# Orange-OpenSource/AIVC

Measured on AMD Instinct MI355X. Metric: encode+decode fps @1080p YUV420 (RA GOP32), higher is better.
Workload: dtype f32; 1 GPU; 1920x1080 8-bit YUV420, coding structure 1_GOP_32: one 128-frame clip = 4 intra-period units of 33 frames (132 coded frames, the last 4 repeat the last frame) encoded + decoded per step; synthetic random-init stand-in for model ms_ssim-4 (widths {'n2': 64, 'n': 128, 'c_y': 64, 'c_short': 64, 'c_z': 32, 'n_h': 128}), last analysis conv calibrated so that 6 (MOFNet) / 12 (CodecNet) of the 64 y featu; parallelism=single GPU

## Files before the change

### aivc_amd/abi.py

```python
import ctypes as C

ABI_VERSION = 23
PREC_FP32, PREC_BF16X3, PREC_FP32_WINO = 0, 1, 2

AIVC_OK = 0
ERR_UNSUPPORTED = -2
ERRORS = {0: 'AIVC_OK', -1: 'AIVC_ERR_ARG', -2: 'AIVC_ERR_UNSUPPORTED', -3: 'AIVC_ERR_LAUNCH',
          -4: 'AIVC_ERR_WORKSPACE'}

MODE_CONV, MODE_TCONV, MODE_GDN, MODE_IGDN = 0, 1, 2, 3
ACT_NONE, ACT_LEAKY, ACT_RELU, ACT_SIGMOID = 0, 1, 2, 3
ALGO_AUTO, ALGO_DIRECT, ALGO_MFMA = 0, 1, 2

AC_MAX_VAL = 256
LP = 514
CDF_ROW = 520
CDF_WIN0, CDF_WIN = 224, 64
BALLE_PARAMS = 43
MAX_MAPS = 256
RC_MAX_STREAMS = 64
RATE_LANES = 16384
SSE_BLOCKS = 64
WINO_MIN_PIXELS = 8000
WINO_MIN_PIXELS_TCONV = 32768
# ... 121 lines not shown
DETMATH_EXPF, DETMATH_EXPM1F, DETMATH_SIGMOIDF, DETMATH_TANHF, DETMATH_SOFTPLUSF = 4, 5, 6, 7, 8
DETMATH_POWF, DETMATH_LAPLACE_CDF = 9, 10
DETMATH_COUNT = 11


def detmath_is_fp64(fn):
    return DETMATH_EXP <= fn <= DETMATH_LOG1P


def detmath_operands(fn):
    return 2 if fn in (DETMATH_POWF, DETMATH_LAPLACE_CDF) else 1

COLOR_PROTOTYPES = {
    'aivc_rgb8_to_yuv420u8': [_f, _i32, _i32, _i32, _f, _f, _f],
    'aivc_yuv8_to_rgb8': [_f, _f, _f, _i32, _i32, _i32, _i32, _i32, _i32, _f],
}

QUALITY_PROTOTYPES = {
    'aivc_frame_sse_u8': [_f, _f, _f, _f, _f, _f, _i32, _i32, _i32, _f, _f],
    'aivc_frame_aux_stats': [_f, _f, _f, _f, _i32, _i32, _i32, _i32, _i32, _i32, _f, _f],
}

RATES_PROTOTYPES = {
    'aivc_channel_gain_rows': [_f, _f, _i32, _sz, _i32, _f],
    'aivc_quantize_center_rows': [_f, _f, _f, _i32, _sz, _i32, _f, _f],
    'aivc_dequantize_rows': [_f, _f, _f, _i32, _sz, _i32, _f],
}

DIGEST_PROTOTYPES = {
    'aivc_md5_batch': [_f, C.c_int64, _i32, _f],
}


def declare(lib, suffix=''):
    fns = {}
    for name, args in PROTOTYPES.items():
        fn = getattr(lib, name + suffix)
        fn.argtypes = list(args) + [C.c_void_p]
        fn.restype = C.c_int
        fns[name] = fn
    if not suffix:
        var = lib.aivc_conv2d_variant
        var.argtypes = [_P(ConvParams)]
        var.restype = C.c_int
        fns['aivc_conv2d_variant'] = var
        chk = lib.aivc_selfcheck_gdn_math
        chk.argtypes = [C.c_uint64, C.c_uint32, _f, C.c_void_p]
        chk.restype = C.c_int
        fns['aivc_selfcheck_gdn_math'] = chk
        ev = lib.aivc_detmath_eval
        ev.argtypes = list(DETMATH_EVAL_ARGS) + [C.c_void_p]
        ev.restype = C.c_int
        fns['aivc_detmath_eval'] = ev
        wm = lib.aivc_warp_modes
        wm.argtypes = [_f, _f, _i32, _i32, _i32, _i32, _i32, _i32, _i32, _f, C.c_void_p]
        wm.restype = C.c_int
        fns['aivc_warp_modes'] = wm
        for name, args in list(COLOR_PROTOTYPES.items()) + list(QUALITY_PROTOTYPES.items()) + list(RATES_PROTOTYPES.items()) \
                + list(DIGEST_PROTOTYPES.items()):
            fn = getattr(lib, name)
            fn.argtypes = list(args) + [C.c_void_p]
            fn.restype = C.c_int
            fns[name] = fn
    mws = getattr(lib, 'aivc_metrics_workspace' + suffix)
    mws.argtypes = [_i32, _i32, _i32]
    mws.restype = C.c_size_t
    fns['aivc_metrics_workspace'] = mws
    ver = getattr(lib, 'aivc_abi_version' + suffix)
    ver.argtypes = []
    ver.restype = C.c_int
    fns['aivc_abi_version'] = ver
    return fns


def conv_out_size(mode, h, w, k, stride, pad):
    if mode == MODE_CONV:
        return (h + 2 * pad - k) // stride + 1, (w + 2 * pad - k) // stride + 1
    if mode == MODE_TCONV:
        return 2 * h, 2 * w
    return h, w
```

### aivc_amd/csrc/conv_wino.hip

```cpp
#include <stdlib.h>

#include "mfma_util.h"
#include "wino_class_walk.h"

namespace aivc {

struct WinoArgs {
  aivc_conv_params p;
  int TH, TW;
  int nby, nbx;
  int gy;
  int total;
  int poly;
  int cpp_shift;
};

constexpr int WINO_RAW_STAGE = 11 * 1024;
constexpr int WINO_U_STAGE = 32 * 1024;
constexpr int WINO_V_QUAD = 1152;
constexpr int WINO_V_POS = 2 * WINO_V_QUAD;
constexpr int WINO_V_STAGE = 16 * WINO_V_POS;
constexpr int WINO_LDS = 2 * (WINO_RAW_STAGE + WINO_U_STAGE + WINO_V_STAGE);

__device__ __attribute__((aligned(4096))) float wino_zeros[1024];

template <int MODE>
__host__ __device__ constexpr bool wino_zero_pos(int pc, int i, int j) {
  if constexpr (MODE == 1) return ((pc >> 1) && i == 3) || ((pc & 1) && j == 3);
  if constexpr (MODE == 2) return ((pc >> 1) && i == 0) || ((pc & 1) && j == 0);
  return false;
}
template <int MODE>
__host__ __device__ constexpr uint32_t wino_pos_mask(int pc, int half) {
  uint32_t m = 0u;
  for (int q = 0; q < 8; ++q) m |= wino_zero_pos<MODE>(pc, 2 * half + (q >> 2), q & 3) ? 0u : 1u << q;
  return m;
}

struct WinoWalk {
  uint32_t x_lo, x_hi, slot, wg_per_xcd;
  __device__ __forceinline__ WinoWalk(uint32_t total, uint32_t nwg, uint32_t wg) {
    const uint32_t xcd = wg & 7u;
    slot = wg >> 3;
    const uint32_t per_xcd = (total + 7u) >> 3;
    wg_per_xcd = (nwg + 7u - xcd) >> 3;
    x_lo = xcd * per_xcd;
    x_hi = min(x_lo + per_xcd, total);
  }
  __device__ __forceinline__ uint32_t block_of(uint32_t k) const { return x_lo + slot + k * wg_per_xcd; }
  __device__ __forceinline__ uint32_t count() const { return x_lo + slot < x_hi ? (x_hi - x_lo - slot + wg_per_xcd - 1u) / wg_per_xcd : 0u; }
};

template <int MODE>
__global__ __launch_bounds__(512) void conv_wino_kernel(WinoArgs a) {
  constexpr bool POLY = MODE == 1, TC = MODE == 2;
  extern __shared__ __attribute__((aligned(16))) char wsmem[];
  char *raw = wsmem, *Us = wsmem + 2 * WINO_RAW_STAGE, *Vs = Us + 2 * WINO_U_STAGE;
  const uint32_t lds0 = (uint32_t)(uintptr_t)(__attribute__((address_space(3))) char *)wsmem;

  const aivc_conv_params &p = a.p;
  const int tid = threadIdx.x, lane = tid & 63;
  const int wave = __builtin_amdgcn_readfirstlane(tid >> 6);
  const int ph = wave >> 2, wm = (wave >> 1) & 1, wn = wave & 1;
  const int H = TC ? p.h_in : p.h_out, W = TC ? p.w_in : p.w_out, Hi = p.h_in, Wi = p.w_in, Cin = p.c_in, Cout = p.c_out;
  const int gyc = TC ? 4 * a.gy : a.gy;
  const int cpp_shift = a.cpp_shift, cpp_mask = (1 << a.cpp_shift) - 1;

  const WinoWalk walk((uint32_t)a.total, gridDim.x, blockIdx.x);
  const uint32_t n_mine = walk.count();
  if (n_mine == 0u) return;
  struct Desc {
    const float *xbase, *ubase;
    uint32_t r_off[2];
    int img, byi, bxi, cb;
  };
  int s_quad[2], s_py[2], s_px[2];
#pragma unroll
  for (int k = 0; k < 2; ++k) {
    int sl = 64 * (wave + 8 * k) + lane;
    sl = sl < 648 ? sl : 647;
    const int q2 = sl >> 1, plane = q2 / 81, rem = q2 - plane * 81, hy = rem / 9, hx = rem - hy * 9;
    s_quad[k] = sl & 1;
    s_py[k] = 2 * hy + (plane >> 1);
    s_px[k] = 2 * hx + (plane & 1);
  }
  const int nch = POLY ? 4 * (Cin >> 3) : (Cin >> 3);
  auto make_desc = [&](uint32_t blk) {
    Desc d;
    uint32_t rest;
    if constexpr (TC) {
      const WinoClassEntry e = wino_class_entry(blk, (uint32_t)gyc, (uint32_t)a.total, gridDim.x);
      d.cb = (int)e.cb;
      rest = e.pb;
    } else {
      d.cb = (int)(blk % (uint32_t)gyc);
      rest = blk / (uint32_t)gyc;
    }
    d.bxi = (int)(rest % (uint32_t)a.nbx);
    rest /= (uint32_t)a.nbx;
    d.byi = (int)(rest % (uint32_t)a.nby);
    d.img = (int)(rest / (uint32_t)a.nby);
    d.xbase = p.x + (size_t)d.img * (size_t)Hi * Wi * Cin;
    d.ubase = p.w_wino + (size_t)d.cb * (size_t)nch * (WINO_U_STAGE / 4);
    if constexpr (MODE == 0) {
#pragma unroll
      for (int k = 0; k < 2; ++k) {
        const int iy = max(min(16 * d.byi - 1 + s_py[k], Hi - 1), 0), ix = max(min(16 * d.bxi - 1 + s_px[k], Wi - 1), 0);
        d.r_off[k] = ((uint32_t)(iy * Wi + ix) * (uint32_t)Cin + (uint32_t)(4 * s_quad[k])) * 4u;
      }
    }
    return d;
  };
  uint32_t iss_off[2];
  auto patch_offsets = [&](const Desc &d_, int ph2) {
    const int st = POLY ? 2 : 1, py = ph2 >> 1, px = ph2 & 1;
#pragma unroll
    for (int k = 0; k < 2; ++k) {
      const int iy = max(min(st * (16 * d_.byi - 1 + s_py[k]) + py, Hi - 1), 0), ix = max(min(st * (16 * d_.bxi - 1 + s_px[k]) + px, Wi - 1), 0);
      iss_off[k] = ((uint32_t)(iy * Wi + ix) * (uint32_t)Cin + (uint32_t)(4 * s_quad[k])) * 4u;
    }
  };
  uint64_t iss_addr[2];
  auto tc_addresses = [&](const Desc &d_) {
#pragma unroll
    for (int k = 0; k < 2; ++k) {
      const int iy = 16 * d_.byi - 1 + s_py[k], ix = 16 * d_.bxi - 1 + s_px[k];
      const bool in = iy >= 0 && iy < Hi && ix >= 0 && ix < Wi;
      const uint64_t a_in = (uint64_t)(uintptr_t)d_.xbase + ((uint64_t)((uint32_t)(iy * Wi + ix)) * (uint32_t)Cin + (uint32_t)(4 * s_quad[k])) * 4u;
      const uint64_t a_z = (uint64_t)(uintptr_t)wino_zeros + (uint32_t)(16 * s_quad[k]);
      iss_addr[k] = in ? a_in : a_z;
    }
  };
  Desc cur = make_desc(walk.block_of(0)), nxt = n_mine > 1u ? make_desc(walk.block_of(1)) : cur;

  const uint32_t r_dst = __builtin_amdgcn_readfirstlane(lds0 + (uint32_t)wave * 1024u);
  const uint32_t u_dst = __builtin_amdgcn_readfirstlane(lds0 + (uint32_t)(2 * WINO_RAW_STAGE) + (uint32_t)wave * 4096u);
  const uint32_t u_off = (uint32_t)(wave * 4096 + lane * 16);
  auto uniform_ptr = [](const float *q) -> const float * {
    const uint64_t v = (uint64_t)(uintptr_t)q;
    const uint32_t lo = __builtin_amdgcn_readfirstlane((uint32_t)v), hi = __builtin_amdgcn_readfirstlane((uint32_t)(v >> 32));
    return reinterpret_cast<const float *>((uintptr_t)(((uint64_t)hi << 32) | lo));
  };
  auto issue_raw = [&](const Desc &d_, int c) {
    const uint32_t d = r_dst + (uint32_t)((c & 1) * WINO_RAW_STAGE);
    if constexpr (TC) {
      if (c == 0) tc_addresses(d_);
      const uint32_t du = __builtin_amdgcn_readfirstlane(d);
      asm volatile("s_mov_b32 m0, %1\n\ts_nop 0\n\tglobal_load_lds_dwordx4 %0, off" : : "v"(iss_addr[0]), "s"(du) : "memory", "m0");
      if (wave < 3) asm volatile("s_mov_b32 m0, %1\n\ts_nop 0\n\tglobal_load_lds_dwordx4 %0, off" : : "v"(iss_addr[1]), "s"(du + 8192u) : "memory", "m0");
      iss_addr[0] += 32u;
      iss_addr[1] += 32u;
    } else {
      const float *src = d_.xbase + 8 * c;
      glds16(src, d_.r_off[0], d);
      if (wave < 3) glds16(src, d_.r_off[1], d + 8192u);
    }
  };
  auto issue_u = [&](const Desc &d_, int c) {
    const float *src = TC ? uniform_ptr(d_.ubase + (size_t)c * (WINO_U_STAGE / 4)) : d_.ubase + (size_t)c * (WINO_U_STAGE / 4);
    const uint32_t d = TC ? __builtin_amdgcn_readfirstlane(u_dst + (uint32_t)((c & 1) * WINO_U_STAGE)) : u_dst + (uint32_t)((c & 1) * WINO_U_STAGE);
    bool lo = true, hi = true;
    if constexpr (TC) {
      const int cls = d_.cb / a.gy, i = wave >> 1, j = 2 * (wave & 1);
      lo = !wino_zero_pos<MODE>(cls, i, j);
      hi = !wino_zero_pos<MODE>(cls, i, j + 1);
    }
    if (lo && hi) glds_piece<GLDS_BOTH>(src, u_off, d);
    else if (lo) glds_piece<GLDS_LO>(src, u_off, d);
    else if (hi) glds_piece<GLDS_HI>(src, u_off, d);
  };

  struct Prep {
    const float *r_src, *u_src;
    uint32_t flags;
  };
  auto prepare = [&](uint32_t kb, int cr, int cu) -> Prep {
    Prep q;
    const bool more = kb + 1u < n_mine;
    uint32_t fl = 0u;
    {
      const bool own = cr < nch;
      const int c = own ? cr : cr - nch;
      const Desc &d_ = own ? cur : nxt;
      if (own || more) {
        fl |= 1u;
        if ((c & cpp_mask) == 0) patch_offsets(d_, c >> cpp_shift);
      }
      q.r_src = uniform_ptr(d_.xbase + 8 * (c & cpp_mask));
    }
    {
      const bool own = cu < nch;
      const int c = own ? cu : cu - nch;
      const Desc &d_ = own ? cur : nxt;
      q.u_src = uniform_ptr(d_.ubase + (size_t)c * (WINO_U_STAGE / 4));
      if (own || more) {
        const int pc = c >> cpp_shift, i = wave >> 1, j = 2 * (wave & 1);
        if (!wino_zero_pos<MODE>(pc, i, j)) fl |= 2u;
        if (!wino_zero_pos<MODE>(pc, i, j + 1)) fl |= 4u;
      }
    }
    q.flags = __builtin_amdgcn_readfirstlane(fl);
    return q;
  };
  auto fire_raw = [&](auto STAGE, const Prep &q) {
    const uint32_t d = r_dst + (uint32_t)(decltype(STAGE)::value * WINO_RAW_STAGE);
    if (q.flags & 1u) {
      glds16(q.r_src, iss_off[0], d);
      if (wave < 3) glds16(q.r_src, iss_off[1], d + 8192u);
    }
  };
  auto fire_u = [&](auto STAGE, const Prep &q) {
    const uint32_t d = u_dst + (uint32_t)(decltype(STAGE)::value * WINO_U_STAGE);
    const uint32_t both = q.flags & 6u;
    if (both == 6u) glds_piece<GLDS_BOTH>(q.u_src, u_off, d);
    else if (both == 2u) glds_piece<GLDS_LO>(q.u_src, u_off, d);
    else if (both == 4u) glds_piece<GLDS_HI>(q.u_src, u_off, d);
  };

  const int l32 = lane & 31;
  const int t_grp = (l32 < 4 || (l32 >= 12 && l32 < 16) || (l32 >= 20 && l32 < 28)) ? 0 : 1;
  const int t_pos = t_grp == 0 ? (l32 < 4 ? l32 : (l32 < 16 ? l32 - 8 : l32 - 12)) : (l32 < 12 ? l32 - 4 : (l32 < 20 ? l32 - 8 : l32 - 16));
  const int t_quad = t_pos >> 3, t_tx = (t_pos & 7) ^ (t_grp << 2), t_ty = ((tid >> 6) & 1) * 4 + (lane >> 5) * 2 + t_grp;
  const int t_i = __builtin_amdgcn_readfirstlane(tid >> 7);
  const int t_ra = t_i == 0 ? 0 : (t_i == 2 ? 2 : 1), t_rb = t_i == 3 ? 3 : (t_i == 2 ? 1 : 2);
  const float t_si = t_i == 1 ? 1.0f : -1.0f;
  const int t_base = ((t_ty * 9 + t_tx) * 2 + t_quad) * 16;
  auto pix_off = [](int r, int c) { return (((r & 1) * 2 + (c & 1)) * 81 + (r >> 1) * 9 + (c >> 1)) * 32; };
  int t_oa[4], t_ob[4];
#pragma unroll
  for (int c = 0; c < 4; ++c) {
    t_oa[c] = t_base + pix_off(t_ra, c);
// ... 75 lines not shown
        const char *rs = raw + (1 - stage) * WINO_RAW_STAGE;
        ta[0] = *reinterpret_cast<const float4 *>(rs + t_oa[st]);
        tb[0] = *reinterpret_cast<const float4 *>(rs + t_ob[st]);
        ta[1] = *reinterpret_cast<const float4 *>(rs + t_oa[st + 1]);
        tb[1] = *reinterpret_cast<const float4 *>(rs + t_ob[st + 1]);
      };
      auto finish = [&](auto S) {
        constexpr int st = decltype(S)::value;
        if constexpr (st < 4) {
          R[st] = comb(ta[0], tb[0], t_si);
          R[st + 1] = comb(ta[1], tb[1], t_si);
        } else {
          transform_step(NEXT{}, integral_constant<int, st>{});
          transform_step(NEXT{}, integral_constant<int, st + 1>{});
        }
      };
      if constexpr (q < 4) reads(Q);
      __builtin_amdgcn_sched_barrier(0);
      const float4 x0 = af[set][0], y0 = bf[set][0], x1 = af[set][1], y1 = bf[set][1];
      if constexpr (first && TC) {
        const floatx16 zero = {0.0f, 0.0f, 0.0f, 0.0f, 0.0f, 0.0f, 0.0f, 0.0f, 0.0f, 0.0f, 0.0f, 0.0f, 0.0f, 0.0f, 0.0f, 0.0f};
        if ((pm >> q) & 1u) acc[q] = mfma_oct1(x0, y0, zero);
        else acc[q] = __builtin_amdgcn_mfma_f32_32x32x2f32(0.0f, 0.0f, zero, 0, 0, 0);
        if ((pm >> (q + 1)) & 1u) acc[q + 1] = mfma_oct1(x1, y1, zero);
        else acc[q + 1] = __builtin_amdgcn_mfma_f32_32x32x2f32(0.0f, 0.0f, zero, 0, 0, 0);
      } else if constexpr (first) {
        const floatx16 zero = {0.0f, 0.0f, 0.0f, 0.0f, 0.0f, 0.0f, 0.0f, 0.0f, 0.0f, 0.0f, 0.0f, 0.0f, 0.0f, 0.0f, 0.0f, 0.0f};
        acc[q] = __builtin_amdgcn_mfma_f32_32x32x2f32(x0.x, y0.x, zero, 0, 0, 0);
        acc[q + 1] = __builtin_amdgcn_mfma_f32_32x32x2f32(x1.x, y1.x, zero, 0, 0, 0);
        acc[q] = __builtin_amdgcn_mfma_f32_32x32x2f32(x0.y, y0.y, acc[q], 0, 0, 0);
        acc[q + 1] = __builtin_amdgcn_mfma_f32_32x32x2f32(x1.y, y1.y, acc[q + 1], 0, 0, 0);
        acc[q] = __builtin_amdgcn_mfma_f32_32x32x2f32(x0.z, y0.z, acc[q], 0, 0, 0);
        acc[q + 1] = __builtin_amdgcn_mfma_f32_32x32x2f32(x1.z, y1.z, acc[q + 1], 0, 0, 0);
        acc[q] = __builtin_amdgcn_mfma_f32_32x32x2f32(x0.w, y0.w, acc[q], 0, 0, 0);
        acc[q + 1] = __builtin_amdgcn_mfma_f32_32x32x2f32(x1.w, y1.w, acc[q + 1], 0, 0, 0);
      } else {
        if (MODE == 0 || ((pm >> q) & 1u)) acc[q] = mfma_oct1(x0, y0, acc[q]);
        if (MODE == 0 || ((pm >> (q + 1)) & 1u)) acc[q + 1] = mfma_oct1(x1, y1, acc[q + 1]);
      }
      __builtin_amdgcn_sched_barrier(0);
      if constexpr (!TC && q == 0) {
        if (!ph) dma();
      }
      finish(Q);
      __builtin_amdgcn_sched_barrier(0);
    };
    using std::integral_constant;
    pair(integral_constant<int, 0>{});
    pair(integral_constant<int, 2>{});
    pair(integral_constant<int, 4>{});
    pair(integral_constant<int, 6>{});
  };

  auto issue_raw_at = [&](uint32_t kb, int c) {
    if (c < nch) issue_raw(cur, c);
    else if (kb + 1u < n_mine) issue_raw(nxt, c - nch);
  };
  auto issue_u_at = [&](uint32_t kb, int c) {
    if (c < nch) issue_u(cur, c);
    else if (kb + 1u < n_mine) issue_u(nxt, c - nch);
  };
  if constexpr (POLY) {
    const Prep q0 = prepare(0u, 0, 0);
    fire_raw(std::integral_constant<int, 0>{}, q0);
    fire_u(std::integral_constant<int, 0>{}, q0);
    fire_raw(std::integral_constant<int, 1>{}, prepare(0u, 1, 0));
  } else {
    issue_raw(cur, 0);
    issue_u(cur, 0);
    issue_raw_at(0u, 1);
  }
  asm volatile("s_waitcnt vmcnt(0)" ::: "memory");
  __builtin_amdgcn_s_barrier();
  transform0();
  asm volatile("s_waitcnt lgkmcnt(0)" ::: "memory");
  __builtin_amdgcn_s_barrier();
  const int act1 = p.act1, act2 = p.act2;
  for (uint32_t kb = 0; kb < n_mine; ++kb) {
    auto chunk = [&](auto STAGE, auto FIRST, int c) {
      Prep q;
      if constexpr (POLY) q = prepare(kb, c + 2, c + 1);
      auto dma = [&]() {
        if constexpr (POLY) {
          fire_raw(STAGE, q);
          fire_u(std::integral_constant<int, 1 - decltype(STAGE)::value>{}, q);
        } else {
          issue_raw_at(kb, c + 2);
          issue_u_at(kb, c + 1);
        }
      };
      uint32_t pm = 0xFFu;
      if constexpr (MODE != 0) {
        constexpr uint32_t ZCOL = 0xFFu ^ wino_pos_mask<MODE>(1, 0), ZROW = 0xFFu ^ wino_pos_mask<MODE>(2, POLY ? 1 : 0);
        static_assert(wino_pos_mask<MODE>(1, 1) == (0xFFu ^ ZCOL) && wino_pos_mask<MODE>(2, POLY ? 0 : 1) == 0xFFu &&
                      wino_pos_mask<MODE>(3, POLY ? 1 : 0) == (0xFFu ^ (ZCOL | ZROW)), "pm's two terms are the whole rule");
        const int pc = POLY ? c >> cpp_shift : cur.cb / a.gy;
        pm = 0xFFu & ~((pc & 1) ? ZCOL : 0u) & ~(((pc >> 1) && (POLY ? ph : !ph)) ? ZROW : 0u);
      }
      if constexpr (TC) dma();
      multiply(STAGE, FIRST, pm, dma);
      asm volatile("s_waitcnt vmcnt(0) lgkmcnt(0)" ::: "memory");
      __builtin_amdgcn_s_barrier();
    };
    {
      using std::integral_constant;
      using S0 = integral_constant<int, 0>;
      using S1 = integral_constant<int, 1>;
      chunk(S0{}, std::true_type{}, 0);
      chunk(S1{}, std::false_type{}, 1);
      for (int c = 2; c < nch; c += 2) {
        chunk(S0{}, std::false_type{}, c);
        chunk(S1{}, std::false_type{}, c + 1);
      }
    }

    floatx16 keep[2], give[2];
    auto fold = [&](auto PH) {
      constexpr int phc = decltype(PH)::value;
#pragma unroll
      for (int bb = 0; bb < 2; ++bb)
#pragma unroll
        for (int r = 0; r < 16; ++r) keep[bb][r] = give[bb][r] = 0.0f;
#pragma unroll
      for (int q = 0; q < 8; ++q) {
        const int i = 2 * phc + (q >> 2), j = q & 3;
        const int t0i = i < 3 ? 1 : 0, t1i = i == 0 ? 0 : (i == 1 ? 1 : -1);
        const int t0j = j < 3 ? 1 : 0, t1j = j == 0 ? 0 : (j == 1 ? 1 : -1);
#pragma unroll
        for (int o = 0; o < 4; ++o) {
          const int cf = ((o >> 1) ? t1i : t0i) * ((o & 1) ? t1j : t0j);
          floatx16 &dst = (o >> 1) == phc ? keep[o & 1] : give[o & 1];
          if (cf > 0) {
#pragma unroll
            for (int r = 0; r < 16; ++r) dst[r] = dst[r] + acc[q][r];
          } else if (cf < 0) {
#pragma unroll
            for (int r = 0; r < 16; ++r) dst[r] = dst[r] - acc[q][r];
          }
        }
      }
    };
    if (ph) fold(std::integral_constant<int, 1>{});
    else fold(std::integral_constant<int, 0>{});
    {
      float *xch = reinterpret_cast<float *>(Vs + WINO_V_STAGE) + wave * 1024;
      const float *theirs = reinterpret_cast<const float *>(Vs + WINO_V_STAGE) + (wave ^ 4) * 1024;
#pragma unroll
      for (int bb = 0; bb < 2; ++bb) {
#pragma unroll
        for (int r = 0; r < 16; ++r) xch[r * 64 + lane] = give[bb][r];
        asm volatile("s_waitcnt lgkmcnt(0)" ::: "memory");
        __builtin_amdgcn_s_barrier();
#pragma unroll
        for (int r = 0; r < 16; ++r) keep[bb][r] = keep[bb][r] + theirs[r * 64 + lane];
        asm volatile("s_waitcnt lgkmcnt(0)" ::: "memory");
        __builtin_amdgcn_s_barrier();
      }
    }

    {
      const float *__restrict__ g_mul = p.mul;
      const float *__restrict__ g_res = p.res;
// ... 54 lines not shown
                if (ok[rr * 2 + b]) *reinterpret_cast<gfloat *>(yb + lane_b + (uint32_t)((2 * rr + b) * 512) * (sx / 512u)) = v;
              }
          }
        };
        using std::integral_constant;
        int kind = -1;
        if (act1 == AIVC_ACT_NONE && act2 == AIVC_ACT_NONE) kind = 0;
        else if (act2 == AIVC_ACT_NONE) kind = act1 == AIVC_ACT_LEAKY ? 1 : 2;
        else if (act1 == AIVC_ACT_NONE) kind = act2 == AIVC_ACT_RELU ? 3 : 4;
        if (kind >= 0 && sx % 512u == 0u) {
          auto go = [&](auto RES, auto INSIDE) {
            switch (kind) {
              case 0: rows(RES, integral_constant<int, 0>{}, INSIDE); break;
              case 1: rows(RES, integral_constant<int, 1>{}, INSIDE); break;
              case 2: rows(RES, integral_constant<int, 2>{}, INSIDE); break;
              case 3: rows(RES, integral_constant<int, 3>{}, INSIDE); break;
              default: rows(RES, integral_constant<int, 4>{}, INSIDE); break;
            }
          };
          if (inside_x) {
            if (g_res) go(integral_constant<bool, true>{}, integral_constant<bool, true>{});
            else go(integral_constant<bool, false>{}, integral_constant<bool, true>{});
          } else {
            if (g_res) go(integral_constant<bool, true>{}, integral_constant<bool, false>{});
            else go(integral_constant<bool, false>{}, integral_constant<bool, false>{});
          }
          goto epilogue_done;
        }
      }
      {
        const size_t ybase = (size_t)cur.img * (size_t)Ho_ * Wo_ * Cout + (size_t)co;
#pragma unroll
        for (int r = 0; r < 16; ++r) {
          const int t = (r & 3) + 8 * (r >> 2) + 4 * hh;
          const int oy = oy_w + 2 * (t >> 3), ox0 = 2 * (8 * cur.bxi + (t & 7));
          if (oy >= H) continue;
#pragma unroll
          for (int b = 0; b < 2; ++b) {
            const int ox = ox0 + b;
            if (ox >= W) continue;
            const size_t o = ybase + ((size_t)(OS * oy + pyc) * Wo_ + (size_t)(OS * ox + pxc)) * (size_t)Cout;
            float v = keep[b][r];
            if (has_bias) v = v + cbias;
            v = act_cheap(act1, v);
            if (g_mul) v = g_mul[o] * v;
            if (g_res) v = v + g_res[o];
            v = act_cheap(act2, v);
            g_y[o] = v;
          }
        }
      }
    epilogue_done:;
    }
    cur = nxt;
    if (kb + 2u < n_mine) nxt = make_desc(walk.block_of(kb + 2u));
  }
}

__device__ __forceinline__ void wino_g(double g0, double g1, double g2, double (&out)[4]) {
  out[0] = g0;
  out[1] = 0.5 * ((g0 + g1) + g2);
  out[2] = 0.5 * ((g0 - g1) + g2);
  out[3] = g2;
}

struct WinoForm3x3 {
  static constexpr int COUNT = 1;
  int co, ci, c_in;
  __device__ WinoForm3x3(size_t idx, int, int c_in_) : co((int)(idx / c_in_)), ci((int)(idx % c_in_)), c_in(c_in_) {}
  __device__ double tap(const float *w, int r, int l) const { return (double)w[(((size_t)co * 3 + r) * 3 + l) * c_in + ci]; }
  __device__ size_t out(int pos) const { return AIVC_WINO_U_INDEX(co, pos, ci, c_in); }
};
__device__ __forceinline__ double wino_tap5(const float *w, int co, int ci, int c_in, int ky, int kx) {
  return ky < 5 && kx < 5 ? (double)w[(((size_t)co * 5 + ky) * 5 + kx) * c_in + ci] : 0.0;
}
struct WinoFormPoly5 {
  static constexpr int COUNT = 4;
  int co, ci, c_in, phase;
  __device__ WinoFormPoly5(size_t idx, int, int c_in_)
      : co((int)(idx / ((size_t)4 * c_in_))), ci((int)((idx / 4) % c_in_)), c_in(c_in_), phase((int)(idx % 4)) {}
  __device__ double tap(const float *w, int r, int l) const { return wino_tap5(w, co, ci, c_in, 2 * r + (phase >> 1), 2 * l + (phase & 1)); }
  __device__ size_t out(int pos) const { return AIVC_WINO_U_INDEX(co, pos, phase * c_in + ci, 4 * c_in); }
};
struct WinoFormTconv5 {
  static constexpr int COUNT = 4;
  int co, ci, c_in, c_out, cls;
  __device__ WinoFormTconv5(size_t idx, int c_out_, int c_in_)
      : co((int)((idx / c_in_) % c_out_)), ci((int)(idx % c_in_)), c_in(c_in_), c_out(c_out_), cls((int)(idx / ((size_t)c_in_ * c_out_))) {}
  __device__ double tap(const float *w, int r, int l) const { return wino_tap5(w, co, ci, c_in, (cls >> 1) + 4 - 2 * r, (cls & 1) + 4 - 2 * l); }
  __device__ size_t out(int pos) const { return AIVC_WINO_U_INDEX(cls * c_out + co, pos, ci, c_in); }
};

template <class FORM>
__global__ void __launch_bounds__(256) winograd_weights_kernel(const float *w, int c_out, int c_in, float *u) {
  const size_t idx = (size_t)blockIdx.x * 256 + threadIdx.x;
  if (idx >= (size_t)c_out * c_in * FORM::COUNT) return;
  const FORM f(idx, c_out, c_in);
  double t[4][3], uu[4][4];
#pragma unroll
  for (int l = 0; l < 3; ++l) {
    double col[4];
    wino_g(f.tap(w, 0, l), f.tap(w, 1, l), f.tap(w, 2, l), col);
#pragma unroll
    for (int i = 0; i < 4; ++i) t[i][l] = col[i];
  }
#pragma unroll
  for (int i = 0; i < 4; ++i) wino_g(t[i][0], t[i][1], t[i][2], uu[i]);
#pragma unroll
  for (int i = 0; i < 4; ++i)
#pragma unroll
    for (int j = 0; j < 4; ++j) u[f.out(4 * i + j)] = (float)uu[i][j];
}

template <class FORM>
static int winograd_weights_launch(const char *what, const float *w, int c_out, int c_in, float *u, hipStream_t s) {
  hipLaunchKernelGGL(winograd_weights_kernel<FORM>, dim3(cdiv((size_t)c_out * c_in * FORM::COUNT, 256)), dim3(256), 0, s, w, c_out, c_in, u);
  return check_launch(what);
}
int winograd_weights(const float *w, int c_out, int c_in, float *u, hipStream_t s) {
  return winograd_weights_launch<WinoForm3x3>("winograd_weights", w, c_out, c_in, u, s);
}
int winograd_weights_poly5(const float *w, int c_out, int c_in, float *u, hipStream_t s) {
  return winograd_weights_launch<WinoFormPoly5>("winograd_weights_poly5", w, c_out, c_in, u, s);
}
int winograd_weights_tconv5(const float *w, int c_out, int c_in, float *u, hipStream_t s) {
  return winograd_weights_launch<WinoFormTconv5>("winograd_weights_tconv5", w, c_out, c_in, u, s);
}

struct WinoGrid {
  int gh, gw, nby, nbx;
  uint64_t blocks;
};
static WinoGrid wino_grid(const aivc_conv_params &p) {
  const bool tc = p.mode == AIVC_MODE_TCONV;
  const int gh = tc ? p.h_in : p.h_out, gw = tc ? p.w_in : p.w_out, nby = (gh + 15) / 16, nbx = (gw + 15) / 16;
  return {gh, gw, nby, nbx, (uint64_t)p.n * nby * nbx * ((uint64_t)p.c_out / 64) * (tc ? 4 : 1)};
}

bool conv2d_wino_supported(const aivc_conv_params &p) {
  if (!aivc_winograd_covers(&p) || p.gdn) return false;
  if ((uint64_t)p.h_in * p.w_in * p.c_in * 4u >= 0xFFFF0000ull) return false;
  if (p.mode == AIVC_MODE_TCONV && p.c_in > 960) return false;
  return wino_grid(p).blocks < 0x7FFFFFFFull;
}

int conv2d_wino_variant(const aivc_conv_params &p) { return p.mode == AIVC_MODE_TCONV ? 303 : (p.ksize == 5 ? 302 : 301); }

template <int MODE>
static int wino_launch(const WinoArgs &a, unsigned grid, hipStream_t s) {
  static LdsOptIn opt_in;
  if (!opt_in.raise(reinterpret_cast<const void *>(conv_wino_kernel<MODE>), WINO_LDS)) return check_launch("conv_wino lds attribute");
  hipLaunchKernelGGL(conv_wino_kernel<MODE>, dim3(grid), dim3(512), WINO_LDS, s, a);
  return check_launch("conv_wino");
}

int conv2d_wino(const aivc_conv_params &p, hipStream_t s) {
  if (!conv2d_wino_supported(p) || !p.w_wino) return AIVC_ERR_UNSUPPORTED;
  const bool tc = p.mode == AIVC_MODE_TCONV;
  WinoArgs a;
  a.p = p;
  a.poly = !tc && p.ksize == 5 ? 1 : 0;
  a.cpp_shift = 0;
  while ((8 << a.cpp_shift) < p.c_in) ++a.cpp_shift;
  const WinoGrid g = wino_grid(p);
  a.TH = (g.gh + 1) / 2;
  a.TW = (g.gw + 1) / 2;
  a.nby = g.nby;
  a.nbx = g.nbx;
  a.gy = p.c_out / 64;
  a.total = (int)g.blocks;
  static std::atomic<int> n_cu{0};
  if (n_cu.load(std::memory_order_relaxed) == 0) {
    int dev = 0, cus = 0;
    n_cu = hipGetDevice(&dev) == hipSuccess && hipDeviceGetAttribute(&cus, hipDeviceAttributeMultiprocessorCount, dev) == hipSuccess && cus > 0 ? cus : 256;
  }
  unsigned grid = (unsigned)n_cu.load(std::memory_order_relaxed);
  if ((unsigned)a.total < grid) grid = (unsigned)a.total;
  if (tc) return wino_launch<2>(a, grid, s);
  return a.poly ? wino_launch<1>(a, grid, s) : wino_launch<0>(a, grid, s);
}

}
```

### aivc_amd/csrc/selfcheck.hip

```cpp
#include "common.h"

namespace aivc {

__global__ __launch_bounds__(256) void selfcheck_sqrt_kernel(uint32_t first, uint32_t last, unsigned long long *bad) {
  unsigned long long n = 0;
  for (uint64_t b = (uint64_t)first + (uint64_t)blockIdx.x * 256 + threadIdx.x; b <= last; b += (uint64_t)gridDim.x * 256) {
    const float s = __uint_as_float((uint32_t)b);
    n += __float_as_uint(sqrt_rn_safe(s)) != __float_as_uint(__builtin_sqrtf(s));
  }
  if (n) atomicAdd(bad, n);
}

__device__ __forceinline__ uint64_t mix64(uint64_t z) {
  z = (z ^ (z >> 30)) * 0xBF58476D1CE4E5B9ull;
  z = (z ^ (z >> 27)) * 0x94D049BB133111EBull;
  return z ^ (z >> 31);
}

__global__ __launch_bounds__(256) void selfcheck_div_kernel(uint64_t n_pairs, uint32_t seed, unsigned long long *bad) {
  unsigned long long n = 0;
  for (uint64_t i = (uint64_t)blockIdx.x * 256 + threadIdx.x; i < n_pairs; i += (uint64_t)gridDim.x * 256) {
    const uint64_t h = mix64(i + ((uint64_t)seed << 32) + 0x9E3779B97F4A7C15ull), h2 = mix64(h);
    const uint32_t ev = 127u - 60u + (uint32_t)((h >> 23) % 120u), ed = 127u - 30u + (uint32_t)((h2 >> 23) % 60u);
    uint32_t mv = (uint32_t)h & 0x7FFFFFu;
    const uint32_t md = (uint32_t)h2 & 0x7FFFFFu;
    if ((i & 3) == 3) mv = (md + (uint32_t)((h >> 50) & 7u) - 3u) & 0x7FFFFFu;
    const float v = __uint_as_float(((uint32_t)(h >> 63) << 31) | (ev << 23) | mv);
    const float d = __uint_as_float((ed << 23) | md);
    n += __float_as_uint(div_rn_safe(v, d)) != __float_as_uint(v / d);
  }
  if (n) atomicAdd(bad, n);
}

}

AIVC_EXPORT int aivc_selfcheck_gdn_math(uint64_t n_div_pairs, uint32_t seed, uint64_t *mismatch, aivc_stream_t stream) {
  if (!mismatch) return AIVC_ERR_ARG;
  hipStream_t s = aivc::to_stream(stream);
  if (hipMemsetAsync(mismatch, 0, 2 * sizeof(uint64_t), s) != hipSuccess) return aivc::check_launch("selfcheck memset");
  const uint32_t first = __builtin_bit_cast(uint32_t, aivc::GDN_SAFE_LO), last = __builtin_bit_cast(uint32_t, aivc::GDN_SAFE_HI);
  hipLaunchKernelGGL(aivc::selfcheck_sqrt_kernel, dim3(4096), dim3(256), 0, s, first, last, reinterpret_cast<unsigned long long *>(mismatch));
  if (n_div_pairs)
    hipLaunchKernelGGL(aivc::selfcheck_div_kernel, dim3(4096), dim3(256), 0, s, n_div_pairs, seed, reinterpret_cast<unsigned long long *>(mismatch) + 1);
  return aivc::check_launch("selfcheck_gdn_math");
}

namespace aivc {

template <typename T>
__global__ __launch_bounds__(256) void detmath_eval_kernel(int fn, const T *__restrict__ a, const T *__restrict__ b, size_t n, T *__restrict__ out) {
  for (size_t i = (size_t)blockIdx.x * 256 + threadIdx.x; i < n; i += (size_t)gridDim.x * 256) {
    if constexpr (sizeof(T) == 8) {
      const double x = a[i];
      double r;
      switch (fn) {
        case AIVC_DETMATH_EXP: r = aivc_det_exp(x); break;
        case AIVC_DETMATH_EXPM1: r = aivc_det_expm1(x); break;
        case AIVC_DETMATH_LOG: r = aivc_det_log(x); break;
        default: r = aivc_det_log1p(x); break;
      }
      out[i] = r;
    } else {
      const float x = a[i];
      float r;
      switch (fn) {
        case AIVC_DETMATH_EXPF: r = aivc_expf_det(x); break;
        case AIVC_DETMATH_EXPM1F: r = aivc_expm1f_det(x); break;
        case AIVC_DETMATH_SIGMOIDF: r = aivc_sigmoidf_det(x); break;
        case AIVC_DETMATH_TANHF: r = aivc_tanhf_det(x); break;
        case AIVC_DETMATH_SOFTPLUSF: r = aivc_softplusf_det(x); break;
        case AIVC_DETMATH_POWF: r = aivc_powf_det(x, b[i]); break;
        default: r = aivc_laplace_cdf(x, b[i]); break;
      }
      out[i] = r;
    }
  }
}

}

AIVC_EXPORT int aivc_detmath_eval(int32_t fn, const void *a, const void *b, size_t n, void *out, aivc_stream_t stream) {
  if (fn < 0 || fn >= AIVC_DETMATH_COUNT) return AIVC_ERR_ARG;
  if (n == 0) return AIVC_OK;
  const bool two = fn == AIVC_DETMATH_POWF || fn == AIVC_DETMATH_LAPLACE_CDF;
  if (!a || !out || (two && !b)) return AIVC_ERR_ARG;
  hipStream_t s = aivc::to_stream(stream);
  const unsigned blocks = aivc::cdiv(n, 256) < 8192u ? aivc::cdiv(n, 256) : 8192u;
  if (fn <= AIVC_DETMATH_LOG1P)
    hipLaunchKernelGGL(aivc::detmath_eval_kernel<double>, dim3(blocks), dim3(256), 0, s, (int)fn, static_cast<const double *>(a),
                       static_cast<const double *>(b), n, static_cast<double *>(out));
  else
    hipLaunchKernelGGL(aivc::detmath_eval_kernel<float>, dim3(blocks), dim3(256), 0, s, (int)fn, static_cast<const float *>(a),
                       static_cast<const float *>(b), n, static_cast<float *>(out));
  return aivc::check_launch("detmath_eval");
}
```

### aivc_amd/ops.py

```python
import ctypes as C
import os

import numpy as np
import torch

from . import abi
from ._lib import AivcNativeError, call, load

FRAME_I, FRAME_P, FRAME_B = abi.FRAME_I, abi.FRAME_P, abi.FRAME_B

PROFILE = None
PROFILE_DIRECT_EQUIVALENT = [0.0, 0.0]
PROFILE_HBM = None


def _hbm_profiled(name, nbytes, launch):
    if PROFILE_HBM is None:
        return launch()
    e0, e1 = torch.cuda.Event(enable_timing=True), torch.cuda.Event(enable_timing=True)
    e0.record()
    launch()
    e1.record()
    PROFILE_HBM.append((name, float(nbytes), e0, e1))

# ... 191 lines not shown
        flags = abi.CONV_SPARSE4 if cmap is not None and all(ci % 4 != 3 for ci in cmap) else 0
        if WINO_ANY_SIZE:
            flags |= abi.CONV_WINO_ANY_SIZE
    ho, wo = abi.conv_out_size(mode, h, w_, k, stride, pad)
    y = torch.empty((n, ho, wo, co2 or co), dtype=torch.float32, device=x.device)
    bias = _dev(bias, torch.float32, 'bias')
    mul = _dev(mul, torch.float32, 'mul')
    res = _dev(res, torch.float32, 'res')
    for t, nm in ((mul, 'mul'), (res, 'res')):
        if t is not None and tuple(t.shape) != tuple(y.shape):
            raise AivcNativeError('conv2d: %s shape %s != output shape %s' % (nm, tuple(t.shape), tuple(y.shape)))
    g_beta, g_gamma, gflag = (None, None, 0) if gdn is None else (gdn[0], gdn[1], 2 if gdn[2] else 1)
    p = abi.ConvParams(mode, k, stride, pad, n, h, w_, c, ho, wo, co, act1, act2, algo, gflag, flags,
                       _p(x), _p(w_ohwi), _p(bias), _p(mul), _p(res), _p(y), _p(g_beta), _p(g_gamma))
    if co2:
        b3 = _dev(tail[1], torch.float32, 'tail bias')
        p.tail_w, p.tail_bias, p.tail_c_out = _p(w3), _p(b3), co2
    p.precision = PRECISION
    if frame_h is not None and PRECISION == abi.PREC_FP32_WINO:
        p.precision, p.flags = slab_contract(p, frame_h)
    variant = load()['aivc_conv2d_variant'](C.byref(p))
    if variant < 0 and (gdn is not None or co2):
        return _two_launches(x, w_ohwi, bias, mode, stride, pad, act1, act2, mul, res, algo, gdn, tail, frame_h)
    w_derived = None
    if variant in _WINO_VARIANTS:
        w_derived = winograd_weights(w_ohwi, transposed=mode == abi.MODE_TCONV)
        p.w_wino = _p(w_derived)
    elif variant >= 1000 and PRESPLIT_WEIGHTS:
        w_derived = split_weights_bf16x3(w_ohwi)
        p.w_bf16x3 = _p(w_derived)
        variant = load()['aivc_conv2d_variant'](C.byref(p))
    _profiled(lambda: call('aivc_conv2d', C.byref(p), _stream()), variant, mode, k, stride, c_real, co, n, h, w_, ho, wo,
              gdn is not None, co2)
    return y


def gdn_reparam(beta, gamma, beta_bound, gamma_bound, pedestal):
    beta = _dev(beta.detach(), torch.float32, 'beta')
    gamma = _dev(gamma.detach(), torch.float32, 'gamma')
    c = beta.shape[0]
    be = torch.empty_like(beta)
    ge = torch.empty_like(gamma)
    call('aivc_gdn_reparam', _p(beta), _p(gamma), c, float(beta_bound), float(gamma_bound),
         float(pedestal), _p(be), _p(ge), _stream())
    return be, ge


def selfcheck_gdn_math(n_div_pairs=1 << 34, seed=1, device=None):
    out = torch.zeros(2, dtype=torch.int64, device=device or torch.device('cuda'))
    call('aivc_selfcheck_gdn_math', int(n_div_pairs), int(seed), _p(out), _stream())
    return tuple(int(v) for v in out.cpu())


def detmath_eval(fn, a, b=None):
    dt = torch.float64 if abi.detmath_is_fp64(fn) else torch.float32
    a, b = _dev(a, dt, 'a'), _dev(b, dt, 'b')
    if abi.detmath_operands(fn) == 2 and (b is None or b.shape != a.shape):
        raise AivcNativeError('aivc_amd.ops.detmath_eval: function %d takes two operands of one shape' % fn)
    out = torch.empty_like(a)
    call('aivc_detmath_eval', int(fn), _p(a), _p(b), a.numel(), _p(out), _stream())
    return out


def gdn(x, beta_eff, gamma_eff, inverse=False, res=None, algo=abi.ALGO_AUTO, frame_h=None):
    c = x.shape[-1]
    mode = abi.MODE_IGDN if inverse else abi.MODE_GDN
    if c % 4 == 0:
        return conv2d(x, gamma_eff.reshape(c, 1, 1, c), beta_eff, mode=mode, res=res, algo=algo, frame_h=frame_h)
    c4 = (c + 3) // 4 * 4
    g = torch.zeros((c4, c4), dtype=torch.float32, device=x.device)
    g[:c, :c] = gamma_eff
    b = torch.ones(c4, dtype=torch.float32, device=x.device)
    b[:c] = beta_eff
    y = conv2d(pad_channels(x, c4), g.reshape(c4, 1, 1, c4), b, mode=mode,
               res=None if res is None else pad_channels(res, c4), algo=algo, frame_h=frame_h)
    return y[..., :c].contiguous()


def yuv420_to_444(y, u, v, c_store=4, c_off=0, out=None):
    u8 = y.dtype == torch.uint8
    dt = torch.uint8 if u8 else torch.float32
    y, u, v = _dev(y, dt, 'y'), _dev(u, dt, 'u'), _dev(v, dt, 'v')
    n, h, w = y.shape
    if out is None:
        full = c_off == 0 and c_store <= 4
        out = (torch.empty if full else torch.zeros)((n, h, w, c_store), dtype=torch.float32, device=y.device)
    zero_pad = 1 if out.shape[-1] >= c_off + 4 else 0
    hc, wc = (h + 1) // 2, (w + 1) // 2
    _hbm_profiled('yuv420_to_444', n * ((h * w + 2 * hc * wc) * (1 if u8 else 4) + h * w * 4 * (3 + zero_pad)),
                  lambda: call('aivc_yuv420u8_to_444' if u8 else 'aivc_yuv420_to_444', _p(y), _p(u), _p(v), n, h, w,
                               _p(out), out.shape[-1], c_off, zero_pad, _stream()))
    return out


_CONV_IMAGES_MAX = 2


def _n_frames(parts):
    return next(p['y'].shape[0] if isinstance(p, dict) else p.shape[0] for p in parts if p is not None)


def _image_sources(parts):
    arr = (abi.ImageSrc * abi.MAX_IMAGES)()
    keep = []
    for i, p in enumerate(parts):
        if isinstance(p, dict):
# ... 664 lines not shown
```

Baseline: 101.8 frames/s.

## Replace static Winograd block walk with per-XCD atomic ticket dynamic scheduling

```diff
diff --git a/aivc_amd/abi.py b/aivc_amd/abi.py
--- a/aivc_amd/abi.py
+++ b/aivc_amd/abi.py
@@ -197,6 +197,10 @@
         ev.argtypes = list(DETMATH_EVAL_ARGS) + [C.c_void_p]
         ev.restype = C.c_int
         fns['aivc_detmath_eval'] = ev
+        hold = lib.aivc_diag_hold_lds
+        hold.argtypes = [C.c_uint32, C.c_uint32, _f, C.c_void_p]
+        hold.restype = C.c_int
+        fns['aivc_diag_hold_lds'] = hold
         wm = lib.aivc_warp_modes
         wm.argtypes = [_f, _f, _i32, _i32, _i32, _i32, _i32, _i32, _i32, _f, C.c_void_p]
         wm.restype = C.c_int
diff --git a/aivc_amd/csrc/conv_wino.hip b/aivc_amd/csrc/conv_wino.hip
--- a/aivc_amd/csrc/conv_wino.hip
+++ b/aivc_amd/csrc/conv_wino.hip
@@ -1,7 +1,11 @@
 #include <stdlib.h>
+
+#include <mutex>
+#include <unordered_map>
 
 #include "mfma_util.h"
 #include "wino_class_walk.h"
+#include "wino_dynamic_walk.h"
 
 namespace aivc {
 
@@ -20,7 +24,11 @@
 constexpr int WINO_V_QUAD = 1152;
 constexpr int WINO_V_POS = 2 * WINO_V_QUAD;
 constexpr int WINO_V_STAGE = 16 * WINO_V_POS;
-constexpr int WINO_LDS = 2 * (WINO_RAW_STAGE + WINO_U_STAGE + WINO_V_STAGE);
+constexpr int WINO_STAGES = 2 * (WINO_RAW_STAGE + WINO_U_STAGE + WINO_V_STAGE);
+constexpr int WINO_LDS = WINO_STAGES + 16;
+
+constexpr unsigned WINO_WALK_SETS = 256;
+__device__ uint32_t wino_walk_slots[WINO_WALK_SETS * WINO_WALK_SLOTS];
 
 __device__ __attribute__((aligned(4096))) float wino_zeros[1024];
 
@@ -38,21 +46,23 @@
 }
 
 struct WinoWalk {
-  uint32_t x_lo, x_hi, slot, wg_per_xcd;
-  __device__ __forceinline__ WinoWalk(uint32_t total, uint32_t nwg, uint32_t wg) {
-    const uint32_t xcd = wg & 7u;
-    slot = wg >> 3;
-    const uint32_t per_xcd = (total + 7u) >> 3;
-    wg_per_xcd = (nwg + 7u - xcd) >> 3;
-    x_lo = xcd * per_xcd;
-    x_hi = min(x_lo + per_xcd, total);
-  }
-  __device__ __forceinline__ uint32_t block_of(uint32_t k) const { return x_lo + slot + k * wg_per_xcd; }
-  __device__ __forceinline__ uint32_t count() const { return x_lo + slot < x_hi ? (x_hi - x_lo - slot + wg_per_xcd - 1u) / wg_per_xcd : 0u; }
+  uint32_t total, set;
+  __device__ __forceinline__ uint32_t claim() const {
+    const uint32_t xcd = blockIdx.x & 7u;
+    uint32_t *ticket = wino_walk_slots + set * WINO_WALK_SLOTS + xcd;
+    return wino_ticket_entry(wino_xcd_range(total, xcd), __hip_atomic_fetch_add(ticket, 1u, __ATOMIC_RELAXED, __HIP_MEMORY_SCOPE_AGENT));
+  }
+  __device__ __forceinline__ void leave() const {
+    uint32_t *set0 = wino_walk_slots + set * WINO_WALK_SLOTS;
+    if (wino_last_out(__hip_atomic_fetch_add(set0 + WINO_WALK_EXIT, 1u, __ATOMIC_RELAXED, __HIP_MEMORY_SCOPE_AGENT), gridDim.x)) {
+#pragma unroll
+      for (uint32_t i = 0; i <= WINO_WALK_EXIT; ++i) __hip_atomic_store(set0 + i, 0u, __ATOMIC_RELAXED, __HIP_MEMORY_SCOPE_AGENT);
+    }
+  }
 };
 
 template <int MODE>
-__global__ __launch_bounds__(512) void conv_wino_kernel(WinoArgs a) {
+__global__ __launch_bounds__(512) void conv_wino_kernel(WinoArgs a, uint32_t walk_set) {
   constexpr bool POLY = MODE == 1, TC = MODE == 2;
   extern __shared__ __attribute__((aligned(16))) char wsmem[];
   char *raw = wsmem, *Us = wsmem + 2 * WINO_RAW_STAGE, *Vs = Us + 2 * WINO_U_STAGE;
@@ -66,9 +76,16 @@
   const int gyc = TC ? 4 * a.gy : a.gy;
   const int cpp_shift = a.cpp_shift, cpp_mask = (1 << a.cpp_shift) - 1;
 
-  const WinoWalk walk((uint32_t)a.total, gridDim.x, blockIdx.x);
-  const uint32_t n_mine = walk.count();
-  if (n_mine == 0u) return;
+  const WinoWalk walk = {(uint32_t)a.total, walk_set};
+  volatile uint32_t *claim_lds = reinterpret_cast<volatile uint32_t *>(wsmem + WINO_STAGES);
+  if (tid == 0) claim_lds[0] = walk.claim();
+  __syncthreads();
+  const uint32_t blk_cur = __builtin_amdgcn_readfirstlane(claim_lds[0]);
+  uint32_t blk_nxt = WINO_WALK_END;
+  if (blk_cur == WINO_WALK_END) {
+    if (tid == 0) walk.leave();
+    return;
+  }
   struct Desc {
     const float *xbase, *ubase;
     uint32_t r_off[2];
@@ -131,7 +148,7 @@
       iss_addr[k] = in ? a_in : a_z;
     }
   };
-  Desc cur = make_desc(walk.block_of(0)), nxt = n_mine > 1u ? make_desc(walk.block_of(1)) : cur;
+  Desc cur = make_desc(blk_cur), nxt = cur;
 
   const uint32_t r_dst = __builtin_amdgcn_readfirstlane(lds0 + (uint32_t)wave * 1024u);
   const uint32_t u_dst = __builtin_amdgcn_readfirstlane(lds0 + (uint32_t)(2 * WINO_RAW_STAGE) + (uint32_t)wave * 4096u);
@@ -174,9 +191,9 @@
     const float *r_src, *u_src;
     uint32_t flags;
   };
-  auto prepare = [&](uint32_t kb, int cr, int cu) -> Prep {
+  auto prepare = [&](int cr, int cu) -> Prep {
     Prep q;
-    const bool more = kb + 1u < n_mine;
+    const bool more = blk_nxt != WINO_WALK_END;
     uint32_t fl = 0u;
     {
       const bool own = cr < nch;
@@ -358,23 +375,23 @@
     pair(integral_constant<int, 6>{});
   };
 
-  auto issue_raw_at = [&](uint32_t kb, int c) {
+  auto issue_raw_at = [&](int c) {
     if (c < nch) issue_raw(cur, c);
-    else if (kb + 1u < n_mine) issue_raw(nxt, c - nch);
-  };
-  auto issue_u_at = [&](uint32_t kb, int c) {
+    else if (blk_nxt != WINO_WALK_END) issue_raw(nxt, c - nch);
+  };
+  auto issue_u_at = [&](int c) {
     if (c < nch) issue_u(cur, c);
-    else if (kb + 1u < n_mine) issue_u(nxt, c - nch);
+    else if (blk_nxt != WINO_WALK_END) issue_u(nxt, c - nch);
   };
   if constexpr (POLY) {
-    const Prep q0 = prepare(0u, 0, 0);
+    const Prep q0 = prepare(0, 0);
     fire_raw(std::integral_constant<int, 0>{}, q0);
     fire_u(std::integral_constant<int, 0>{}, q0);
-    fire_raw(std::integral_constant<int, 1>{}, prepare(0u, 1, 0));
+    fire_raw(std::integral_constant<int, 1>{}, prepare(1, 0));
   } else {
     issue_raw(cur, 0);
     issue_u(cur, 0);
-    issue_raw_at(0u, 1);
+    issue_raw_at(1);
   }
   asm volatile("s_waitcnt vmcnt(0)" ::: "memory");
   __builtin_amdgcn_s_barrier();
@@ -382,17 +399,17 @@
   asm volatile("s_waitcnt lgkmcnt(0)" ::: "memory");
   __builtin_amdgcn_s_barrier();
   const int act1 = p.act1, act2 = p.act2;
-  for (uint32_t kb = 0; kb < n_mine; ++kb) {
+  for (;;) {
     auto chunk = [&](auto STAGE, auto FIRST, int c) {
       Prep q;
-      if constexpr (POLY) q = prepare(kb, c + 2, c + 1);
+      if constexpr (POLY) q = prepare(c + 2, c + 1);
       auto dma = [&]() {
         if constexpr (POLY) {
           fire_raw(STAGE, q);
           fire_u(std::integral_constant<int, 1 - decltype(STAGE)::value>{}, q);
         } else {
-          issue_raw_at(kb, c + 2);
-          issue_u_at(kb, c + 1);
+          issue_raw_at(c + 2);
+          issue_u_at(c + 1);
         }
       };
       uint32_t pm = 0xFFu;
@@ -412,8 +429,13 @@
       using std::integral_constant;
       using S0 = integral_constant<int, 0>;
       using S1 = integral_constant<int, 1>;
+      uint32_t ahead = WINO_WALK_END;
+      if (tid == 0) ahead = walk.claim();
       chunk(S0{}, std::true_type{}, 0);
+      if (tid == 0) claim_lds[0] = ahead;
       chunk(S1{}, std::false_type{}, 1);
+      blk_nxt = __builtin_amdgcn_readfirstlane(claim_lds[0]);
+      if (blk_nxt != WINO_WALK_END) nxt = make_desc(blk_nxt);
       for (int c = 2; c < nch; c += 2) {
         chunk(S0{}, std::false_type{}, c);
         chunk(S1{}, std::false_type{}, c + 1);
@@ -574,9 +596,10 @@
       }
     epilogue_done:;
     }
+    if (blk_nxt == WINO_WALK_END) break;
     cur = nxt;
-    if (kb + 2u < n_mine) nxt = make_desc(walk.block_of(kb + 2u));
-  }
+  }
+  if (tid == 0) walk.leave();
 }
 
 __device__ __forceinline__ void wino_g(double g0, double g1, double g2, double (&out)[4]) {
@@ -668,11 +691,35 @@
 
 int conv2d_wino_variant(const aivc_conv_params &p) { return p.mode == AIVC_MODE_TCONV ? 303 : (p.ksize == 5 ? 302 : 301); }
 
+static int wino_walk_set(hipStream_t s) {
+  static std::mutex mu;
+  static std::unordered_map<hipStream_t, unsigned> set_of;
+  std::lock_guard<std::mutex> lock(mu);
+  const auto it = set_of.find(s);
+  if (it != set_of.end()) return (int)it->second;
+  unsigned set = (unsigned)set_of.size();
+  if (set >= WINO_WALK_SETS) {
+    auto idle = set_of.begin();
+    while (idle != set_of.end() && hipStreamQuery(idle->first) == hipErrorNotReady) ++idle;
+    (void)hipGetLastError();
+    if (idle == set_of.end()) return -1;
+    set = idle->second;
+    set_of.erase(idle);
+  }
+  set_of.emplace(s, set);
+  return (int)set;
+}
+
 template <int MODE>
 static int wino_launch(const WinoArgs &a, unsigned grid, hipStream_t s) {
   static LdsOptIn opt_in;
   if (!opt_in.raise(reinterpret_cast<const void *>(conv_wino_kernel<MODE>), WINO_LDS)) return check_launch("conv_wino lds attribute");
-  hipLaunchKernelGGL(conv_wino_kernel<MODE>, dim3(grid), dim3(512), WINO_LDS, s, a);
+  const int set = wino_walk_set(s);
+  if (set < 0) {
+    set_last_error("conv_wino: more streams with launches in flight than block-walk slot sets");
+    return AIVC_ERR_LAUNCH;
+  }
+  hipLaunchKernelGGL(conv_wino_kernel<MODE>, dim3(grid), dim3(512), WINO_LDS, s, a, (uint32_t)set);
   return check_launch("conv_wino");
 }
 
diff --git a/aivc_amd/csrc/selfcheck.hip b/aivc_amd/csrc/selfcheck.hip
--- a/aivc_amd/csrc/selfcheck.hip
+++ b/aivc_amd/csrc/selfcheck.hip
@@ -1,4 +1,6 @@
 #include "common.h"
+
+#include "../../include/aivc_hip_diag.h"
 
 namespace aivc {
 
@@ -94,3 +96,24 @@
                        static_cast<const float *>(b), n, static_cast<float *>(out));
   return aivc::check_launch("detmath_eval");
 }
+
+namespace aivc {
+
+__global__ __launch_bounds__(64) void hold_lds_kernel(uint32_t words, uint32_t iterations, uint32_t *__restrict__ out) {
+  extern __shared__ uint32_t held[];
+  for (uint32_t i = threadIdx.x; i < words; i += 64u) held[i] = i;
+  __syncthreads();
+  uint32_t at = threadIdx.x % words;
+  for (uint32_t k = 0; k < iterations; ++k) at = (held[at] * 2654435761u + k) % words;
+  out[threadIdx.x] = at;
+}
+
+}
+
+AIVC_EXPORT int aivc_diag_hold_lds(uint32_t lds_bytes, uint32_t iterations, uint32_t *out, aivc_stream_t stream) {
+  if (!out || lds_bytes < 256u || lds_bytes > 160u * 1024u || (lds_bytes & 3u) || iterations < 1u || iterations > (1u << 20)) return AIVC_ERR_ARG;
+  static aivc::LdsOptIn opt_in;
+  if (!opt_in.raise(reinterpret_cast<const void *>(aivc::hold_lds_kernel), 160u * 1024u)) return aivc::check_launch("diag_hold_lds lds attribute");
+  hipLaunchKernelGGL(aivc::hold_lds_kernel, dim3(1), dim3(64), lds_bytes, aivc::to_stream(stream), lds_bytes / 4u, iterations, out);
+  return aivc::check_launch("diag_hold_lds");
+}
diff --git a/aivc_amd/csrc/wino_dynamic_walk.h b/aivc_amd/csrc/wino_dynamic_walk.h
--- /dev/null
+++ b/aivc_amd/csrc/wino_dynamic_walk.h
@@ -0,0 +1,33 @@
+#pragma once
+#include <stdint.h>
+
+#if defined(__HIPCC__) || defined(__CUDACC__)
+#define AIVC_WINO_WALK_HD __host__ __device__
+#else
+#define AIVC_WINO_WALK_HD
+#endif
+
+namespace aivc {
+
+constexpr uint32_t WINO_WALK_XCDS = 8u;
+constexpr uint32_t WINO_WALK_EXIT = 8u;
+constexpr uint32_t WINO_WALK_SLOTS = 16u;
+constexpr uint32_t WINO_WALK_END = 0xFFFFFFFFu;
+
+struct WinoXcdRange {
+  uint32_t lo, hi;
+};
+
+AIVC_WINO_WALK_HD inline WinoXcdRange wino_xcd_range(uint32_t total, uint32_t xcd) {
+  const uint32_t per_xcd = (total + 7u) >> 3, lo = xcd * per_xcd;
+  const uint32_t hi = lo + per_xcd < total ? lo + per_xcd : total;
+  return {lo, hi > lo ? hi : lo};
+}
+
+AIVC_WINO_WALK_HD inline uint32_t wino_ticket_entry(WinoXcdRange r, uint32_t ticket) {
+  return ticket < r.hi - r.lo ? r.lo + ticket : WINO_WALK_END;
+}
+
+AIVC_WINO_WALK_HD inline bool wino_last_out(uint32_t exits_before, uint32_t nwg) { return exits_before + 1u == nwg; }
+
+}
diff --git a/aivc_amd/ops.py b/aivc_amd/ops.py
--- a/aivc_amd/ops.py
+++ b/aivc_amd/ops.py
@@ -267,6 +267,13 @@
     return tuple(int(v) for v in out.cpu())
 
 
+def diag_hold_lds(lds_bytes, iterations, out=None):
+    if out is None:
+        out = torch.empty(64, dtype=torch.int32, device=torch.device('cuda'))
+    call('aivc_diag_hold_lds', int(lds_bytes), int(iterations), _p(out), _stream())
+    return out
+
+
 def detmath_eval(fn, a, b=None):
     dt = torch.float64 if abi.detmath_is_fp64(fn) else torch.float32
     a, b = _dev(a, dt, 'a'), _dev(b, dt, 'b')
diff --git a/include/aivc_hip_diag.h b/include/aivc_hip_diag.h
--- /dev/null
+++ b/include/aivc_hip_diag.h
@@ -0,0 +1,16 @@
+#ifndef AIVC_HIP_DIAG_H
+#define AIVC_HIP_DIAG_H
+
+#include "aivc_hip.h"
+
+#ifdef __cplusplus
+extern "C" {
+#endif
+
+int aivc_diag_hold_lds(uint32_t lds_bytes, uint32_t iterations, uint32_t *out, aivc_stream_t stream);
+
+#ifdef __cplusplus
+}
+#endif
+
+#endif
```

Measured after the change: 103.8 frames/s (median of 6 runs). +2.0%, better.
